# jrkerns/pylinac

Measured on AMD Instinct MI355X. Metric: EPID images/s, filter->threshold->profile->peak on 1024^2 batch, higher is better.
Workload: dtype f64

## Files before the change

pylinac_amd/csrc/hist_otsu.hip:

```cpp
#include "pl_common.h"
#include "median3_rows.h"

constexpr int kOtsuAhead = 2;

namespace {

constexpr int kHistThreads = 1024;

template <int PARTS, bool RUNS>
__global__ void __launch_bounds__(kHistThreads)
hist16_kernel(const unsigned short* __restrict__ in, int64_t n, int64_t count, unsigned flip,
              uint32_t* __restrict__ hist, const int32_t* __restrict__ only ,
              unsigned virtual_blocks) {
  constexpr int kBins = 65536 / PARTS;
  constexpr int kShift = PARTS == 4 ? 14 : 15;
  extern __shared__ unsigned bins[];
  if (only) {
    int any = 0;
    for (int64_t i = threadIdx.x; i < n; i += kHistThreads) any |= only[i];
    if (!__syncthreads_or(any)) return;
  }
  for (unsigned vb = blockIdx.x; vb < virtual_blocks; vb += gridDim.x) {
  const unsigned within = vb % (8 * PARTS);
  const int64_t frame = (int64_t)(vb / (8 * PARTS)) * 8 + (within & 7);
  const unsigned part = within >> 3;
  if (frame >= n) continue;
  if (only && !only[frame]) continue;
  __syncthreads();
  for (int i = threadIdx.x; i < kBins; i += kHistThreads) bins[i] = 0;
  __syncthreads();

  const unsigned short* src = in + frame * count;
  unsigned prev = 0xffffffffu, run = 0;
  auto tally = [&](unsigned key) {
    key ^= flip;
    if constexpr (RUNS) {
      const unsigned b = ((key >> kShift) == part) ? (key & (kBins - 1)) : 0xffffffffu;
      if (b == prev) {
        ++run;
      } else {
        if (prev != 0xffffffffu) atomicAdd(&bins[prev], run);
        prev = b;
        run = 1;
      }
    } else {
      if ((key >> kShift) == part) atomicAdd(&bins[key & (kBins - 1)], 1u);
    }
  };
  if ((reinterpret_cast<uintptr_t>(src) & 15) == 0) {
    const int64_t nvec = count / 8;
    const uint4* vsrc = reinterpret_cast<const uint4*>(src);
    auto tally4 = [&](uint4 q) {
      const unsigned first = q.x & 0xffffu;
      const unsigned splat = first | (first << 16);
      const bool lane_flat = q.x == splat && q.y == splat && q.z == splat && q.w == splat;
      const unsigned wave_first = __builtin_amdgcn_readfirstlane(splat);
      const unsigned long long active = __ballot(1);
      if (__ballot(!(lane_flat && splat == wave_first)) == 0) {
        if constexpr (!RUNS) {
          const unsigned key = (wave_first & 0xffffu) ^ flip;
          if ((key >> kShift) == part && (threadIdx.x & 63) == __builtin_ctzll(active))
            atomicAdd(&bins[key & (kBins - 1)], 8u * (unsigned)__popcll(active));
          return;
        }
      }
      const unsigned wds[4] = {q.x, q.y, q.z, q.w};
#pragma unroll
      for (int k = 0; k < 4; ++k) {
        tally(wds[k] & 0xffffu);
        tally(wds[k] >> 16);
      }
    };
    int64_t v = threadIdx.x;
    constexpr int U = 4;
    for (; v + (int64_t)(U - 1) * kHistThreads < nvec; v += (int64_t)U * kHistThreads) {
      uint4 q[U];
#pragma unroll
      for (int k = 0; k < U; ++k) q[k] = vsrc[v + (int64_t)k * kHistThreads];
#pragma unroll
      for (int k = 0; k < U; ++k) tally4(q[k]);
    }
    for (; v < nvec; v += kHistThreads) tally4(vsrc[v]);
    for (int64_t i = nvec * 8 + threadIdx.x; i < count; i += kHistThreads) tally(src[i]);
  } else {
    for (int64_t i = threadIdx.x; i < count; i += kHistThreads) tally(src[i]);
  }
  if constexpr (RUNS) {
    if (prev != 0xffffffffu) atomicAdd(&bins[prev], run);
  }
  __syncthreads();
  uint32_t* dst = hist + frame * 65536 + (size_t)part * kBins;
  for (int i = threadIdx.x; i < kBins; i += kHistThreads) dst[i] = bins[i];
  }
}

template <int PARTS, bool RUNS>
int launch_hist16(const unsigned short* in, int64_t n, int64_t count, unsigned flip, uint32_t* hist, hipStream_t st,
                  const int32_t* only = nullptr) {
  const size_t lds = (size_t)(65536 / PARTS) * sizeof(unsigned);
  static std::atomic<bool> attr{false};
  if (!attr) {
    if (hipFuncSetAttribute((const void*)hist16_kernel<PARTS, RUNS>, hipFuncAttributeMaxDynamicSharedMemorySize,
                            (int)lds) != hipSuccess) {
      (void)hipGetLastError();
      return -1;
    }
    attr = true;
  }
  const int64_t blocks = pl_cdiv(n, 8) * 8 * PARTS;
  if (blocks > 0x7fffffffLL) return -1;
  const unsigned grid = only ? (unsigned)(blocks < 256 ? blocks : 256) : (unsigned)blocks;
  hipLaunchKernelGGL((hist16_kernel<PARTS, RUNS>), dim3(grid), dim3(kHistThreads), lds, st, in, n, count,
                     flip, hist, only, (unsigned)blocks);
  return 0;
}

struct Pair { unsigned long long c; long long s; };

__device__ __forceinline__ Pair block_exclusive_scan(Pair v, Pair* total, Pair* wave_tot ) {
  const int lane = threadIdx.x & 63, wv = threadIdx.x >> 6;
  Pair inc = v;
#pragma unroll
  for (int o = 1; o < 64; o <<= 1) {
    unsigned long long c = __shfl_up(inc.c, o, 64);
    long long s = __shfl_up(inc.s, o, 64);
    if (lane >= o) { inc.c += c; inc.s += s; }
  }
  if (lane == 63) wave_tot[wv] = inc;
  __syncthreads();
  Pair base = {0, 0};
  Pair tot = {0, 0};
  for (int k = 0; k < kHistThreads / 64; ++k) {
    if (k < wv) { base.c += wave_tot[k].c; base.s += wave_tot[k].s; }
    tot.c += wave_tot[k].c; tot.s += wave_tot[k].s;
  }
  __syncthreads();
  *total = tot;
  Pair ex = {base.c + inc.c - v.c, base.s + inc.s - v.s};
  return ex;
}

__global__ void __launch_bounds__(kHistThreads)
otsu_kernel(const uint32_t* __restrict__ hist, int bias, int32_t* __restrict__ thr,
            int32_t* __restrict__ vmin, int32_t* __restrict__ vmax, const int32_t* __restrict__ only) {
  __shared__ Pair wave_tot[kHistThreads / 64];
  __shared__ int s_lo[kHistThreads / 64], s_hi[kHistThreads / 64];
  __shared__ double s_var[kHistThreads / 64];
  __shared__ int s_idx[kHistThreads / 64];
  const int64_t frame = blockIdx.x;
  if (only && !only[frame]) return;
  const uint32_t* hh = hist + frame * 65536;
  const int b0 = threadIdx.x * 64;
  const uint4* p = reinterpret_cast<const uint4*>(hh + b0);
  Pair mine = {0, 0};
  int lo = 1 << 30, hi = -1;
  for (int k4 = 0; k4 < 16; ++k4) {
    const uint4 q = p[k4];
    const uint32_t c[4] = {q.x, q.y, q.z, q.w};
#pragma unroll
    for (int j = 0; j < 4; ++j) {
      const int b = b0 + 4 * k4 + j;
      mine.c += c[j];
      mine.s += (long long)c[j] * (long long)(b - bias);
      if (c[j]) { if (lo == (1 << 30)) lo = b; hi = b; }
    }
  }
  lo = pl_wave_reduce(lo, [](int a, int b) { return a < b ? a : b; });
  hi = pl_wave_reduce(hi, [](int a, int b) { return a > b ? a : b; });
  const int lane = threadIdx.x & 63, wv = threadIdx.x >> 6;
  if (lane == 0) { s_lo[wv] = lo; s_hi[wv] = hi; }
  Pair total;
  Pair ex = block_exclusive_scan(mine, &total, wave_tot);
  for (int k = 0; k < kHistThreads / 64; ++k) { lo = s_lo[k] < lo ? s_lo[k] : lo; hi = s_hi[k] > hi ? s_hi[k] : hi; }

  double best = -1.0;
  int best_k = 1 << 30;
  double dw1 = (double)ex.c, ds1 = (double)ex.s;
  const double dW = (double)total.c, dS = (double)total.s;
  for (int k4 = 0; k4 < 16; ++k4) {
    const uint4 q = p[k4];
    const uint32_t c[4] = {q.x, q.y, q.z, q.w};
#pragma unroll
    for (int j = 0; j < 4; ++j) {
      const int b = b0 + 4 * k4 + j;
      if (c[j] != 0u) {
        dw1 += (double)c[j];
        ds1 = fma((double)c[j], (double)(b - bias), ds1);
        if (b >= lo && b < hi) {
          const double dw2 = dW - dw1;
          const double m1 = ds1 / dw1;
          const double m2 = (dS - ds1) / dw2;
          const double d = m1 - m2;
          const double var = (dw1 * dw2) * (d * d);
          if (var > best) { best = var; best_k = b; }
        }
      }
    }
  }
#pragma unroll
  for (int o = 32; o > 0; o >>= 1) {
    double ov = __shfl_xor(best, o, 64);
    int ok = __shfl_xor(best_k, o, 64);
    if (ov > best || (ov == best && ok < best_k)) { best = ov; best_k = ok; }
  }
  if (lane == 0) { s_var[wv] = best; s_idx[wv] = best_k; }
  __syncthreads();
  if (threadIdx.x == 0) {
    for (int k = 1; k < kHistThreads / 64; ++k)
      if (s_var[k] > best || (s_var[k] == best && s_idx[k] < best_k)) { best = s_var[k]; best_k = s_idx[k]; }
    thr[frame] = (lo == hi) ? (lo - bias) : (best_k - bias);
    if (vmin) vmin[frame] = lo - bias;
    if (vmax) vmax[frame] = hi - bias;
  }
}

constexpr int kWinBins = 38912;
struct OtsuScratch {
  Pair wave_tot[kHistThreads / 64];
  double s_var[kHistThreads / 64];
  int s_lo[kHistThreads / 64], s_hi[kHistThreads / 64], s_idx[kHistThreads / 64];
  int any;
};
constexpr int kOtsuScratchAt = ((kWinBins + 1) * 4 + 15) & ~15;
constexpr size_t kOtsuLds = kOtsuScratchAt + sizeof(OtsuScratch);

__device__ __forceinline__ int cell_max_see(int cm, const int (&m)[8]) {
  cm = max(max(cm, m[0]), m[1]);
  cm = max(max(cm, m[2]), m[3]);
  cm = max(max(cm, m[4]), m[5]);
  return max(max(cm, m[6]), m[7]);
}
__device__ __forceinline__ void cell_max_store(unsigned short* __restrict__ row_cells, int cm, int lane, bool on) {
  const unsigned g = pl_group8_max(on ? (unsigned)cm : 0u);
  if (on && (lane & 7) == 0) row_cells[lane >> 3] = (unsigned short)g;
}

template <typename T, bool MED3, bool CELLS>
__global__ void __launch_bounds__(kHistThreads)
otsu16_window_kernel(const unsigned short* __restrict__ in, int64_t count, int h, int w, unsigned flip, int bias,
                     const int32_t* __restrict__ lo_hint, const int32_t* __restrict__ hi_hint, int32_t* __restrict__ thr,
                     int32_t* __restrict__ vmin, int32_t* __restrict__ vmax, int32_t* __restrict__ flag, int parts,
                     uint32_t* __restrict__ merge ,
                     unsigned short* __restrict__ cellmax) {
  extern __shared__ __attribute__((aligned(16))) unsigned bins[];
  OtsuScratch& scr = *reinterpret_cast<OtsuScratch*>(reinterpret_cast<unsigned char*>(bins) + kOtsuScratchAt);
  Pair* const wave_tot = scr.wave_tot;
  int* const s_lo = scr.s_lo;
  int* const s_hi = scr.s_hi;
  double* const s_var = scr.s_var;
  int* const s_idx = scr.s_idx;
  const int64_t frame = blockIdx.x / (unsigned)parts;
  const int part = (int)(blockIdx.x % (unsigned)parts);
  const unsigned short* src = in + frame * count;
  const int lane = threadIdx.x & 63, wv = threadIdx.x >> 6;
  int klo, khi;
  if (lo_hint) {
    klo = lo_hint[frame] + bias;
    khi = hi_hint[frame] + bias;
  } else {
    int mn = 1 << 30, mx = -1;
    auto see = [&](unsigned key) {
      const int k = (int)(key ^ flip);
      mn = k < mn ? k : mn;
      mx = k > mx ? k : mx;
    };
    if ((reinterpret_cast<uintptr_t>(src) & 15) == 0 && count >= 8) {
      const int64_t nvec = count / 8;
      const uint4* vsrc = reinterpret_cast<const uint4*>(src);
      for (int64_t blk = threadIdx.x >> 7; blk * 2048 < nvec; blk += kHistThreads >> 7) {
        const int64_t idx = blk * 2048 + (threadIdx.x & 127);
        if (idx < nvec) {
          const uint4 q = vsrc[idx];
          const unsigned wds[4] = {q.x, q.y, q.z, q.w};
#pragma unroll
          for (int k = 0; k < 4; ++k) { see(wds[k] & 0xffffu); see(wds[k] >> 16); }
        }
      }
    } else {
      for (int64_t i = threadIdx.x; i < count; i += 16LL * kHistThreads) see(src[i]);
    }
    mn = pl_wave_reduce(mn, [](int a, int b) { return a < b ? a : b; });
    mx = pl_wave_reduce(mx, [](int a, int b) { return a > b ? a : b; });
    if (lane == 0) { s_lo[wv] = mn; s_hi[wv] = mx; }
    __syncthreads();
    for (int k = 0; k < kHistThreads / 64; ++k) { mn = s_lo[k] < mn ? s_lo[k] : mn; mx = s_hi[k] > mx ? s_hi[k] : mx; }
    __syncthreads();
    if (mx < mn) { mn = 0; mx = 0; }
    const int slack = kWinBins - (mx - mn + 1);
    klo = mn - (slack > 0 ? slack / 2 : 0);
    if (klo < 0) klo = 0;
    khi = klo + kWinBins - 1;
    if (khi > 65535) { khi = 65535; klo = khi - kWinBins + 1; }
    if (slack < 0) khi = klo + kWinBins;
  }
  const int range = khi - klo + 1;
  if (range > kWinBins || range <= 0 || klo < 0 || khi > 65535 || (MED3 && pl_lds_base(bins) != 0u)) {
    if (threadIdx.x == 0) flag[frame] = 1;
    return;
  }
  for (int i = threadIdx.x; i <= range; i += kHistThreads) bins[i] = 0;
  if (threadIdx.x == 0) scr.any = 0;
  __syncthreads();

  int outside = 0;
  auto tally = [&](unsigned key) {
    const unsigned b = (key ^ flip) - (unsigned)klo;
    if (b < (unsigned)range) atomicAdd(&bins[b], 1u);
    else outside = 1;
  };
  if (MED3) {
    constexpr int kRows = 32;
    constexpr int kSBias = ((T)-1 < (T)0) ? 32768 : 0;
    const unsigned kbase4 = 4u * (unsigned)(kSBias - klo);
    const int col_waves = (w / 8 + PL_WAVE - 1) / PL_WAVE, row_groups = (h + kRows - 1) / kRows;
    const int rg_lo = (int)((int64_t)row_groups * part / parts), rg_hi = (int)((int64_t)row_groups * (part + 1) / parts);
    for (int item = rg_lo * col_waves + __builtin_amdgcn_readfirstlane(wv); item < col_waves * rg_hi; item += kHistThreads / 64) {
      const int c0 = ((item % col_waves) * PL_WAVE + lane) * 8;
      const bool on = c0 < w;
      const unsigned long long act = __ballot(on);
      if (act == 0ull) continue;
      const int first_on = __builtin_ctzll(act);
      const unsigned cap4 = on ? 4u * (unsigned)range : 0u;
      const unsigned inc = on ? 1u : 0u;
      int cm = 0;
      pl_median3_rows<T, kRows, kOtsuAhead>(reinterpret_cast<const T*>(src), h, w, c0, lane, (item / col_waves) * kRows,
                             [&](int, const int (&m)[8]) {
        if constexpr (CELLS) cm = cell_max_see(cm, m);
        unsigned spread = 0;
#pragma unroll
        for (int k = 1; k < 8; ++k) spread |= (unsigned)(m[k] ^ m[0]);
        const int wave_first = __builtin_amdgcn_readlane(m[0], first_on);
        if (__ballot(on && (spread | (unsigned)(m[0] ^ wave_first)) != 0u) == 0ull) {
          const unsigned b = (unsigned)(wave_first + kSBias - klo);
          if (b < (unsigned)range) {
            if (lane == first_on) atomicAdd(&bins[b], 8u * (unsigned)__popcll(act));
          } else {
            outside = 1;
          }
          return;
        }
#pragma unroll
        for (int k = 0; k < 8; ++k) {
          const unsigned b4 = ((unsigned)m[k] << 2) + kbase4;
          const unsigned a4 = b4 < cap4 ? b4 : cap4;
          pl_lds_add_abs(a4, inc);
        }
      });
      if constexpr (CELLS) {
        const int cell_cols = (w + 63) / 64;
        cell_max_store(cellmax + ((size_t)frame * row_groups + item / col_waves) * cell_cols + (item % col_waves) * (PL_WAVE / 8), cm,
                       lane, on);
      }
    }
  } else if ((reinterpret_cast<uintptr_t>(src) & 15) == 0) {
    const int64_t nvec = count / 8;
    const uint4* vsrc = reinterpret_cast<const uint4*>(src);
    auto tally4 = [&](uint4 q) {
      const unsigned first = q.x & 0xffffu;
      const unsigned splat = first | (first << 16);
      const bool lane_flat = q.x == splat && q.y == splat && q.z == splat && q.w == splat;
      const unsigned wave_first = __builtin_amdgcn_readfirstlane(splat);
      const unsigned long long active = __ballot(1);
      if (__ballot(!(lane_flat && splat == wave_first)) == 0) {
        const unsigned b = ((wave_first & 0xffffu) ^ flip) - (unsigned)klo;
        if (b < (unsigned)range) {
          if ((threadIdx.x & 63) == __builtin_ctzll(active)) atomicAdd(&bins[b], 8u * (unsigned)__popcll(active));
        } else {
          outside = 1;
        }
        return;
      }
      const unsigned wds[4] = {q.x, q.y, q.z, q.w};
#pragma unroll
      for (int k = 0; k < 4; ++k) {
        tally(wds[k] & 0xffffu);
        tally(wds[k] >> 16);
      }
    };
    const int64_t v_lo = nvec * part / parts, v_hi = nvec * (part + 1) / parts;
    int64_t v = v_lo + threadIdx.x;
    constexpr int U = 4;
    for (; v + (int64_t)(U - 1) * kHistThreads < v_hi; v += (int64_t)U * kHistThreads) {
      uint4 q[U];
#pragma unroll
      for (int k = 0; k < U; ++k) q[k] = vsrc[v + (int64_t)k * kHistThreads];
#pragma unroll
      for (int k = 0; k < U; ++k) tally4(q[k]);
    }
    for (; v < v_hi; v += kHistThreads) tally4(vsrc[v]);
    if (part == parts - 1)
      for (int64_t i = nvec * 8 + threadIdx.x; i < count; i += kHistThreads) tally(src[i]);
  } else {
    const int64_t i_lo = count * part / parts, i_hi = count * (part + 1) / parts;
    for (int64_t i = i_lo + threadIdx.x; i < i_hi; i += kHistThreads) tally(src[i]);
  }
  if (outside) scr.any = 1;
  __syncthreads();
  const bool spilled = scr.any != 0 || (MED3 && bins[range] != 0u);
  if (parts == 1) {
    if (spilled) {
      if (threadIdx.x == 0) flag[frame] = 1;
      return;
    }
    if (threadIdx.x == 0) flag[frame] = 0;
  } else {
    uint32_t* table = merge + frame * 65536;
    unsigned seen = 0;
    if (spilled && threadIdx.x == 0) seen |= atomicExch(&flag[frame], 1) == 0x7fffffff ? 1u : 0u;
    if (!spilled)
      for (int i = threadIdx.x; i < range; i += kHistThreads) {
        const unsigned c = bins[i];
        if (c) seen |= atomicAdd(&table[i], c) == 0xffffffffu ? 1u : 0u;
      }
    if (seen) scr.any = 2;
    __syncthreads();
    if (threadIdx.x == 0) scr.any = atomicAdd(&table[65534], scr.any == 2 ? 0u : 1u) == (unsigned)(parts - 1) ? 1 : 0;
    __syncthreads();
    if (scr.any == 0) return;
    if (__hip_atomic_load(&flag[frame], __ATOMIC_RELAXED, __HIP_MEMORY_SCOPE_AGENT) != 0) return;
    for (int i = threadIdx.x; i < range; i += kHistThreads)
      bins[i] = __hip_atomic_load(&table[i], __ATOMIC_RELAXED, __HIP_MEMORY_SCOPE_AGENT);
    __syncthreads();
  }

  const int per = ((range + kHistThreads - 1) / kHistThreads) | 1;
  const int b0 = threadIdx.x * per;
  const int b1 = b0 + per < range ? b0 + per : range;
  Pair mine = {0, 0};
  int lo = 1 << 30, hi = -1;
  for (int b = b0; b < b1; ++b) {
    const unsigned c = bins[b];
    mine.c += c;
    mine.s += (long long)c * (long long)(b + klo - bias);
    if (c) { if (lo == (1 << 30)) lo = b; hi = b; }
  }
  lo = pl_wave_reduce(lo, [](int a, int b) { return a < b ? a : b; });
  hi = pl_wave_reduce(hi, [](int a, int b) { return a > b ? a : b; });
  if (lane == 0) { s_lo[wv] = lo; s_hi[wv] = hi; }
  Pair total;
  Pair ex = block_exclusive_scan(mine, &total, wave_tot);
  for (int k = 0; k < kHistThreads / 64; ++k) { lo = s_lo[k] < lo ? s_lo[k] : lo; hi = s_hi[k] > hi ? s_hi[k] : hi; }

  double best = -1.0;
  int best_k = 1 << 30;
  double dw1 = (double)ex.c, ds1 = (double)ex.s;
  const double dW = (double)total.c, dS = (double)total.s;
  for (int b = b0; b < b1; ++b) {
    const unsigned c = bins[b];
    if (c != 0u) {
      dw1 += (double)c;
      ds1 = fma((double)c, (double)(b + klo - bias), ds1);
      if (b >= lo && b < hi) {
        const double dw2 = dW - dw1;
        const double m1 = ds1 / dw1;
        const double m2 = (dS - ds1) / dw2;
        const double d = m1 - m2;
        const double var = (dw1 * dw2) * (d * d);
        if (var > best) { best = var; best_k = b; }
      }
    }
  }
#pragma unroll
  for (int o = 32; o > 0; o >>= 1) {
    double ov = __shfl_xor(best, o, 64);
    int ok = __shfl_xor(best_k, o, 64);
    if (ov > best || (ov == best && ok < best_k)) { best = ov; best_k = ok; }
  }
  if (lane == 0) { s_var[wv] = best; s_idx[wv] = best_k; }
  __syncthreads();
  if (threadIdx.x == 0) {
    for (int k = 1; k < kHistThreads / 64; ++k)
      if (s_var[k] > best || (s_var[k] == best && s_idx[k] < best_k)) { best = s_var[k]; best_k = s_idx[k]; }
    thr[frame] = (lo == hi) ? (lo + klo - bias) : (best_k + klo - bias);
    if (vmin) vmin[frame] = lo + klo - bias;
    if (vmax) vmax[frame] = hi + klo - bias;
  }
}

constexpr int kFullEvents = 2048;
constexpr int kFullBulk = 64;
struct FullScratch {
  Pair wave_tot[kHistThreads / 64];
  double s_var[kHistThreads / 64];
  int s_lo[kHistThreads / 64], s_hi[kHistThreads / 64], s_idx[kHistThreads / 64];
  int n_events, n_bulk;
  unsigned bulk_key[kFullBulk], bulk_cnt[kFullBulk];
  unsigned short event_key[kFullEvents];
};
constexpr int kFullBinsBytes = 65536 * 2;
constexpr size_t kFullLds = kFullBinsBytes + sizeof(FullScratch);

template <typename T, bool MED3, bool GUARD, bool CELLS>
__device__ __forceinline__ void full_tally_pass(const unsigned short* __restrict__ src, int64_t count, int h, int w, unsigned flip,
                                                unsigned* __restrict__ bins, FullScratch& scr,
                                                unsigned short* __restrict__ frame_cells) {
  const int lane = threadIdx.x & 63, wv = threadIdx.x >> 6;
  auto tally_n = [&](unsigned key, unsigned n) {
    const unsigned sh = (key >> 15) << 4, at = key & 0x7fffu;
    if (!GUARD) {
      pl_lds_add_abs((key << 2) & 0x1fffcu, n * (1u + ((key >> 15) & 1u) * 0xffffu));
      return;
    }
    const unsigned old = atomicAdd(&bins[at], n << sh);
    const unsigned f = (old >> sh) & 0xffffu;
    if (f < 0x8000u && f + n >= 0x8000u) {
      atomicSub(&bins[at], 0x8000u << sh);
      const int slot = atomicAdd(&scr.n_events, 1);
      if (slot < kFullEvents) scr.event_key[slot] = (unsigned short)key;
    }
  };
  auto tally = [&](unsigned key) { tally_n(key, 1u); };
  auto tally_bulk = [&](unsigned key, unsigned n, int first_on) {
    if (GUARD) {
      if (lane == first_on) tally_n(key, n);
      return;
    }
    const int have = scr.n_bulk < kFullBulk ? scr.n_bulk : kFullBulk;
    const unsigned long long hit = __ballot(lane < have && scr.bulk_key[lane] == key);
    if (lane != first_on) return;
    if (hit) { atomicAdd(&scr.bulk_cnt[__builtin_ctzll(hit)], n); return; }
    const int slot = atomicAdd(&scr.n_bulk, 1);
    if (slot < kFullBulk) { atomicAdd(&scr.bulk_cnt[slot], n); scr.bulk_key[slot] = key; }
    else tally_n(key, n);
  };
  if (MED3) {
    constexpr int kRows = 32;
    constexpr int kSBias = ((T)-1 < (T)0) ? 32768 : 0;
    const int col_waves = (w / 8 + PL_WAVE - 1) / PL_WAVE, row_groups = (h + kRows - 1) / kRows;
    for (int item = __builtin_amdgcn_readfirstlane(wv); item < col_waves * row_groups; item += kHistThreads / 64) {
      const int c0 = ((item % col_waves) * PL_WAVE + lane) * 8;
      const bool on = c0 < w;
      const unsigned long long act = __ballot(on);
      if (act == 0ull) continue;
      const int first_on = __builtin_ctzll(act);
      int cm = 0;
      pl_median3_rows<T, kRows, kOtsuAhead>(reinterpret_cast<const T*>(src), h, w, c0, lane, (item / col_waves) * kRows,
                             [&](int, const int (&m)[8]) {
        if constexpr (CELLS) cm = cell_max_see(cm, m);
        unsigned spread = 0;
#pragma unroll
        for (int k = 1; k < 8; ++k) spread |= (unsigned)(m[k] ^ m[0]);
        const int wave_first = __builtin_amdgcn_readlane(m[0], first_on);
        if (__ballot(on && (spread | (unsigned)(m[0] ^ wave_first)) != 0u) == 0ull) {
          tally_bulk((unsigned)(wave_first + kSBias), 8u * (unsigned)__popcll(act), first_on);
          return;
        }
        if (!on) return;
#pragma unroll
        for (int k = 0; k < 8; ++k) tally((unsigned)(m[k] + kSBias));
      });
      if constexpr (CELLS)
        cell_max_store(frame_cells + (size_t)(item / col_waves) * ((w + 63) / 64) + (item % col_waves) * (PL_WAVE / 8), cm, lane, on);
    }
  } else {
    for (int64_t i = threadIdx.x; i < count; i += kHistThreads) tally((unsigned)src[i] ^ flip);
  }
}

template <typename T, bool MED3, bool CELLS>
__global__ void __launch_bounds__(kHistThreads)
otsu16_full_kernel(const unsigned short* __restrict__ in, int64_t count, int h, int w, unsigned flip, int bias,
                   int32_t* __restrict__ thr, int32_t* __restrict__ vmin, int32_t* __restrict__ vmax,
                   int32_t* __restrict__ flag, unsigned short* __restrict__ cellmax) {
  extern __shared__ __attribute__((aligned(16))) unsigned bins[];
  FullScratch& scr = *reinterpret_cast<FullScratch*>(reinterpret_cast<unsigned char*>(bins) + kFullBinsBytes);
  const int64_t frame = blockIdx.x;
  if (flag[frame] == 0) return;
  const unsigned short* src = in + frame * count;
  unsigned short* frame_cells = CELLS ? cellmax + (size_t)frame * ((h + 31) / 32) * ((w + 63) / 64) : nullptr;
  const int lane = threadIdx.x & 63, wv = threadIdx.x >> 6;
  auto clear = [&]() {
    for (int i = threadIdx.x; i < 32768; i += kHistThreads) bins[i] = 0;
    if (threadIdx.x < kFullBulk) { scr.bulk_key[threadIdx.x] = 0xffffffffu; scr.bulk_cnt[threadIdx.x] = 0; }
    if (threadIdx.x == 0) { scr.n_events = 0; scr.n_bulk = 0; }
    __syncthreads();
  };

  const int b0 = threadIdx.x * 64;
  int n_events = 0, n_bulk = 0, my_notes = 0;
  auto count_of = [&](int b) {
    unsigned c = (bins[b & 0x7fff] >> ((b >> 15) << 4)) & 0xffffu;
    if (my_notes) {
      for (int e = 0; e < n_events; ++e) c += (int)scr.event_key[e] == b ? 32768u : 0u;
      for (int e = 0; e < n_bulk; ++e) c += (int)scr.bulk_key[e] == b ? scr.bulk_cnt[e] : 0u;
    }
    return c;
  };
  Pair mine, total, ex, wrapped;
  int lo, hi;
  auto totals = [&]() {
    n_events = scr.n_events < kFullEvents ? scr.n_events : kFullEvents;
    n_bulk = scr.n_bulk < kFullBulk ? scr.n_bulk : kFullBulk;
    my_notes = 0;
    for (int e = 0; e < n_events; ++e) my_notes += ((int)scr.event_key[e] >> 6) == (int)threadIdx.x ? 1 : 0;
    for (int e = 0; e < n_bulk; ++e) my_notes += (scr.bulk_key[e] >> 6) == threadIdx.x ? 1 : 0;
    mine = {0, 0};
    wrapped = {0, 0};
    lo = 1 << 30, hi = -1;
    for (int j = 0; j < 64; ++j) {
      const int b = b0 + ((j + lane) & 63);
      const unsigned c = count_of(b);
      Pair& acc = j + lane < 64 ? mine : wrapped;
      acc.c += c;
      acc.s += (long long)c * (long long)(b - bias);
      if (c) { lo = b < lo ? b : lo; hi = b > hi ? b : hi; }
    }
    mine.c += wrapped.c;
    mine.s += wrapped.s;
    lo = pl_wave_reduce(lo, [](int a, int b) { return a < b ? a : b; });
    hi = pl_wave_reduce(hi, [](int a, int b) { return a > b ? a : b; });
    if (lane == 0) { scr.s_lo[wv] = lo; scr.s_hi[wv] = hi; }
    ex = block_exclusive_scan(mine, &total, scr.wave_tot);
    for (int k = 0; k < kHistThreads / 64; ++k) { lo = scr.s_lo[k] < lo ? scr.s_lo[k] : lo; hi = scr.s_hi[k] > hi ? scr.s_hi[k] : hi; }
  };

  bool exact = false;
  if (pl_lds_base(bins) == 0u) {
    clear();
    full_tally_pass<T, MED3, false, CELLS>(src, count, h, w, flip, bins, scr, frame_cells);
    __syncthreads();
    totals();
    exact = total.c == (unsigned long long)count;
    __syncthreads();
  }
  if (!exact) {
    clear();
    full_tally_pass<T, MED3, true, CELLS>(src, count, h, w, flip, bins, scr, frame_cells);
    __syncthreads();
    totals();
  }
  double best = -1.0;
  int best_k = 1 << 30;
  double dw1 = (double)(ex.c + wrapped.c);
  double ds1 = (double)(ex.s + wrapped.s);
  const double dW = (double)total.c, dS = (double)total.s;
  for (int j = 0; j < 64; ++j) {
    if (j + lane == 64) { dw1 = (double)ex.c; ds1 = (double)ex.s; }
    const int b = b0 + ((j + lane) & 63);
    const unsigned c = count_of(b);
    if (c != 0u) {
      dw1 += (double)c;
      ds1 = fma((double)c, (double)(b - bias), ds1);
      if (b >= lo && b < hi) {
        const double dw2 = dW - dw1;
        const double m1 = ds1 / dw1;
        const double m2 = (dS - ds1) / dw2;
        const double d = m1 - m2;
        const double var = (dw1 * dw2) * (d * d);
        if (var > best || (var == best && b < best_k)) { best = var; best_k = b; }
      }
    }
  }
#pragma unroll
  for (int o = 32; o > 0; o >>= 1) {
    double ov = __shfl_xor(best, o, 64);
    int ok = __shfl_xor(best_k, o, 64);
    if (ov > best || (ov == best && ok < best_k)) { best = ov; best_k = ok; }
  }
  if (lane == 0) { scr.s_var[wv] = best; scr.s_idx[wv] = best_k; }
  __syncthreads();
  if (threadIdx.x == 0) {
    for (int k = 1; k < kHistThreads / 64; ++k)
      if (scr.s_var[k] > best || (scr.s_var[k] == best && scr.s_idx[k] < best_k)) { best = scr.s_var[k]; best_k = scr.s_idx[k]; }
    thr[frame] = (lo == hi) ? (lo - bias) : (best_k - bias);
    if (vmin) vmin[frame] = lo - bias;
    if (vmax) vmax[frame] = hi - bias;
  }
}

__global__ void __launch_bounds__(kHistThreads)
order_stats_kernel(const uint32_t* __restrict__ hist, int bias, const int64_t* __restrict__ ranks,
                   int nranks, int32_t* __restrict__ out) {
  __shared__ Pair wave_tot[kHistThreads / 64];
  const int64_t frame = blockIdx.x;
  const uint32_t* hh = hist + frame * 65536;
  const int b0 = threadIdx.x * 64;
  Pair mine = {0, 0};
  for (int k = 0; k < 64; ++k) mine.c += hh[b0 + k];
  Pair total;
  Pair ex = block_exclusive_scan(mine, &total, wave_tot);
  for (int q = 0; q < nranks; ++q) {
    long long r = ranks[q];
    if (r < 0) r = 0;
    if ((unsigned long long)r >= total.c) r = (long long)total.c - 1;
    if ((unsigned long long)r >= ex.c && (unsigned long long)r < ex.c + mine.c) {
      unsigned long long acc = ex.c;
      for (int k = 0; k < 64; ++k) {
        acc += hh[b0 + k];
        if ((unsigned long long)r < acc) { out[frame * nranks + q] = b0 + k - bias; break; }
      }
    }
  }
}


constexpr int kTwBinsWide = 19456, kTwBinsWl = 9728;
struct TwScratch { int s_lo[kHistThreads / 64], s_hi[kHistThreads / 64]; };
constexpr int tw_scratch_at(int bins) { return (2 * bins + 1 + PL_WAVE + 3) / 4 * 16; }
constexpr size_t tw_lds(int bins) { return tw_scratch_at(bins) + sizeof(TwScratch); }

template <int kTwBins, int WAVES_PER_EU>
__global__ void __launch_bounds__(kHistThreads, WAVES_PER_EU)
hist16_two_window_kernel(const unsigned short* __restrict__ in, int64_t count, unsigned flip, uint32_t* __restrict__ hist,
                         unsigned short* __restrict__ tile_max , int eh, int ew, int ews,
                         int32_t* __restrict__ edge_min, int32_t* __restrict__ edge_max ,
                         const int64_t* __restrict__ ranks, int nranks, int32_t* __restrict__ stats ) {
  extern __shared__ __attribute__((aligned(16))) unsigned bins[];
  TwScratch& scr = *reinterpret_cast<TwScratch*>(reinterpret_cast<unsigned char*>(bins) + tw_scratch_at(kTwBins));
  const int64_t frame = blockIdx.x;
  const unsigned short* src = in + frame * count;
  uint32_t* row = hist + frame * 65536;
  const int lane = threadIdx.x & 63, wv = threadIdx.x >> 6;
  const bool vec = (reinterpret_cast<uintptr_t>(src) & 15) == 0 && count >= 8;
  const int64_t nvec = vec ? count / 8 : 0;
  const uint4* vsrc = reinterpret_cast<const uint4*>(src);

  for (int i = threadIdx.x; i < 2 * kTwBins; i += kHistThreads) bins[i] = 0;
  if (edge_min) {
    int mn = 0x7fffffff, mx = -0x7fffffff - 1;
    auto value = [&](unsigned short raw) { return flip ? (int)(short)raw : (int)raw; };
    auto see = [&](int v) { mn = v < mn ? v : mn; mx = v > mx ? v : mx; };
    const int band = ews < eh ? ews : eh, cb = ews < ew ? ews : ew;
    constexpr int E = 4;
    for (int e0 = threadIdx.x; e0 < band * ew; e0 += E * kHistThreads) {
      unsigned short a[E], b[E];
#pragma unroll
      for (int k = 0; k < E; ++k) {
        const int e = e0 + k * kHistThreads < band * ew ? e0 + k * kHistThreads : e0;
        a[k] = src[e];
        b[k] = src[(int64_t)(eh - band) * ew + e];
      }
#pragma unroll
      for (int k = 0; k < E; ++k) { see(value(a[k])); see(value(b[k])); }
    }
    for (int e0 = threadIdx.x; e0 < eh * cb; e0 += E * kHistThreads) {
      unsigned short a[E], b[E];
#pragma unroll
      for (int k = 0; k < E; ++k) {
        const int e = e0 + k * kHistThreads < eh * cb ? e0 + k * kHistThreads : e0;
        const int r = e / cb, c = e - r * cb;
        a[k] = src[(int64_t)r * ew + c];
        b[k] = src[(int64_t)r * ew + (ew - cb) + c];
      }
#pragma unroll
      for (int k = 0; k < E; ++k) { see(value(a[k])); see(value(b[k])); }
    }
    mn = pl_wave_reduce(mn, [](int a, int b) { return a < b ? a : b; });
    mx = pl_wave_reduce(mx, [](int a, int b) { return a > b ? a : b; });
    if (lane == 0) { scr.s_lo[wv] = mn; scr.s_hi[wv] = mx; }
    __syncthreads();
    if (threadIdx.x == 0) {
      for (int k = 0; k < kHistThreads / 64; ++k) { mn = scr.s_lo[k] < mn ? scr.s_lo[k] : mn; mx = scr.s_hi[k] > mx ? scr.s_hi[k] : mx; }
      edge_min[frame] = mn;
      edge_max[frame] = mx;
    }
    __syncthreads();
  }
  const int64_t ntiles = (count + 511) / 512;
  unsigned short* const tmax = tile_max ? tile_max + frame * ntiles : nullptr;
  if (tmax)
    for (int64_t i = threadIdx.x; i < ntiles; i += kHistThreads) tmax[i] = (unsigned short)0xffffu;
  int mn = 1 << 30, mx = -1;
  auto see = [&](unsigned key) {
    const int k = (int)(key ^ flip);
    mn = k < mn ? k : mn;
    mx = k > mx ? k : mx;
  };
  if (vec) {
    for (int64_t blk = threadIdx.x >> 7; blk * 2048 < nvec; blk += kHistThreads >> 7) {
      const int64_t idx = blk * 2048 + (threadIdx.x & 127);
      if (idx < nvec) {
        const uint4 q = vsrc[idx];
        const unsigned wds[4] = {q.x, q.y, q.z, q.w};
#pragma unroll
        for (int k = 0; k < 4; ++k) { see(wds[k] & 0xffffu); see(wds[k] >> 16); }
      }
    }
  } else {
    for (int64_t i = threadIdx.x; i < count; i += 16LL * kHistThreads) see(src[i]);
  }
  mn = pl_wave_reduce(mn, [](int a, int b) { return a < b ? a : b; });
  mx = pl_wave_reduce(mx, [](int a, int b) { return a > b ? a : b; });
  if (lane == 0) { scr.s_lo[wv] = mn; scr.s_hi[wv] = mx; }
  __syncthreads();
  for (int k = 0; k < kHistThreads / 64; ++k) { mn = scr.s_lo[k] < mn ? scr.s_lo[k] : mn; mx = scr.s_hi[k] > mx ? scr.s_hi[k] : mx; }
  if (mx < mn) { mn = 0; mx = 0; }
  int w0, w1;
  if (mx - mn + 1 <= 2 * kTwBins) {
    w0 = mn - (2 * kTwBins - (mx - mn + 1)) / 2;
    w0 = w0 < 0 ? 0 : (w0 > 65536 - 2 * kTwBins ? 65536 - 2 * kTwBins : w0);
    w1 = w0 + kTwBins;
  } else {
    w0 = mn - 256 < 0 ? 0 : mn - 256;
    w1 = mx + 256 > 65535 ? 65536 - kTwBins : mx + 257 - kTwBins;
    if (w1 < w0 + kTwBins) w1 = w0 + kTwBins;
  }
  const unsigned uw0 = (unsigned)w0, uw1 = (unsigned)w1;
  for (int i = threadIdx.x; i < 65536 / 4; i += kHistThreads) {
    const unsigned b = 4u * (unsigned)i;
    const bool inside = (b - uw0 < (unsigned)kTwBins && b + 3u - uw0 < (unsigned)kTwBins) ||
                        (b - uw1 < (unsigned)kTwBins && b + 3u - uw1 < (unsigned)kTwBins);
    if (!inside) reinterpret_cast<uint4*>(row)[i] = uint4{0u, 0u, 0u, 0u};
  }
  __syncthreads();

  unsigned hot = 0;
  unsigned guess = 0xffffffffu;
  auto add_key = [&](unsigned key, unsigned n) {
    const unsigned b0 = key - uw0, b1 = key - uw1;
    if (b0 < (unsigned)kTwBins) atomicAdd(&bins[b0], n);
    else if (b1 < (unsigned)kTwBins) atomicAdd(&bins[kTwBins + b1], n);
    else atomicAdd(row + key, n);
  };
  auto flush = [&]() {
    const unsigned tot = pl_wave_reduce(hot, [](unsigned a, unsigned b) { return a + b; });
    if (tot != 0u && lane == 0) add_key(guess, tot);
    hot = 0;
    return tot;
  };
  const unsigned base = pl_lds_base(bins);
  const unsigned k0 = base - 4u * uw0, k1 = base + 4u * (unsigned)kTwBins - 4u * uw1;
  const unsigned spare_addr = base + 4u * (unsigned)(2 * kTwBins), dummy_addr = spare_addr + 4u + 4u * (unsigned)lane;
  auto tally = [&](unsigned raw, unsigned long long& outside) {
    const unsigned key = raw ^ flip;
    const bool in0 = key - uw0 < (unsigned)kTwBins, in1 = key - uw1 < (unsigned)kTwBins, is_hot = key == guess;
    unsigned addr = in0 ? (key << 2) + k0 : (in1 ? (key << 2) + k1 : spare_addr);
    addr = is_hot ? dummy_addr : addr;
    hot += is_hot ? 1u : 0u;
    pl_lds_add_abs(addr, 1u);
    outside |= __ballot(!(in0 || in1 || is_hot));
  };
  auto tally4 = [&](uint4 q) {
    const unsigned first = q.x & 0xffffu;
    const unsigned splat = first | (first << 16);
    const bool lane_flat = q.x == splat && q.y == splat && q.z == splat && q.w == splat;
    const unsigned wave_first = __builtin_amdgcn_readfirstlane(splat);
    const unsigned long long active = __ballot(1);
    if (__ballot(!(lane_flat && splat == wave_first)) == 0) {
      if ((threadIdx.x & 63) == __builtin_ctzll(active)) add_key((wave_first & 0xffffu) ^ flip, 8u * (unsigned)__popcll(active));
// ... 364 lines not shown
```

pylinac_amd/csrc/median3_rows.h:

```cpp
#pragma once

template <typename T, int ROWS, int AHEAD = 4, bool BYOFFSET = false, typename F>
__device__ __forceinline__ void pl_median3_rows(const T* __restrict__ f, int h, int w, int c0, int lane, int r0_lane, F&& consume,
                                                bool load = true) {
  static_assert(sizeof(T) == 2, "16-bit dtypes");
  const int r0 = __builtin_amdgcn_readfirstlane(r0_lane);
  const bool active = c0 < w;
  const unsigned offc = (unsigned)(active ? c0 : 0) * 2u;
  const bool first = c0 == 0, last = c0 + 8 >= w;
  const bool edge_l = lane == 0 && !first, edge_r = lane == PL_WAVE - 1 && !last && active;
  const bool edge = edge_l || edge_r;
  const unsigned offe = edge_l ? offc - 2u : offc + 16u;
  struct Raw { uint4 q; int e; };
  [[maybe_unused]] __amdgpu_buffer_rsrc_t rs;
  [[maybe_unused]] unsigned voffq = 0, voffe = 0;
  if constexpr (BYOFFSET) {
    rs = pl_make_rsrc_bounded(f, (unsigned)h * (unsigned)w * 2u);
    voffq = load ? offc : kPlBufferNowhere;
    voffe = load && edge ? offe : kPlBufferNowhere;
  }
  auto fetch = [&](int r) {
    const int rm = 2 * h - 1 - r;
    int rr = r < rm ? r : rm;
    rr = rr > 0 ? rr : 0;
    const char* row = reinterpret_cast<const char*>(f) + (size_t)rr * (size_t)w * 2u;
    Raw x{uint4{0u, 0u, 0u, 0u}, 0};
    if constexpr (BYOFFSET) {
      const unsigned soff = (unsigned)rr * (unsigned)w * 2u;
      x.q = pl_buffer_load_u128(rs, voffq, soff);
      x.e = (int)pl_buffer_load_u16(rs, voffe, soff);
    } else if (load) {
      x.q = *reinterpret_cast<const uint4*>(row + offc);
      x.e = edge ? (int)*reinterpret_cast<const T*>(row + offe) : 0;
    }
    return x;
  };
  int lo[3][8], mi[3][8], hi[3][8];
  auto digest = [&](const Raw& x, int slot) {
    const unsigned wd[4] = {x.q.x, x.q.y, x.q.z, x.q.w};
    int xe = x.e;
    if constexpr (BYOFFSET) xe = pl_extend16_here<T>(x.e);
    int v[10];
#pragma unroll
    for (int k = 0; k < 4; ++k) {
      v[1 + 2 * k] = (int)(T)(wd[k] & 0xffffu);
      v[2 + 2 * k] = (int)(T)(wd[k] >> 16);
    }
    const int left = __builtin_amdgcn_update_dpp(xe, v[8], 0x138, 0xf, 0xf, false);
    const int right = __builtin_amdgcn_update_dpp(xe, v[1], 0x130, 0xf, 0xf, false);
    v[0] = first ? v[1] : left;
    v[9] = last ? v[8] : right;
#pragma unroll
    for (int j = 0; j < 8; ++j) {
      const int a = v[j], b = v[j + 1], c = v[j + 2];
      lo[slot][j] = min(min(a, b), c);
      hi[slot][j] = max(max(a, b), c);
      mi[slot][j] = pl_smed3(a, b, c);
    }
  };
  auto emit = [&](int k) {
    const int r = r0 + k - 2;
    if (r >= h) return;
    int m[8];
#pragma unroll
    for (int j = 0; j < 8; ++j)
      m[j] = pl_smed3(max(max(lo[0][j], lo[1][j]), lo[2][j]), pl_smed3(mi[0][j], mi[1][j], mi[2][j]),
                      min(min(hi[0][j], hi[1][j]), hi[2][j]));
    consume(r, m);
  };
  Raw ring[AHEAD];
#pragma unroll
  for (int k = 0; k < AHEAD; ++k) ring[k] = fetch(r0 - 1 + k);
  constexpr int kChunk = (AHEAD % 3 == 0) ? AHEAD : 3 * AHEAD;
  auto step = [&](int k, int ring_slot, int tri_slot) {
    const Raw cur = ring[ring_slot];
    ring[ring_slot] = fetch(r0 - 1 + k + AHEAD);
    digest(cur, tri_slot);
  };
  step(0, 0 % AHEAD, 0);
  step(1, 1 % AHEAD, 1);
  constexpr int kMain = (ROWS / kChunk) * kChunk;
#pragma unroll 1
  for (int kb = 2; kb < 2 + kMain; kb += kChunk) {
#pragma unroll
    for (int j = 0; j < kChunk; ++j) {
      step(kb + j, (2 + j) % AHEAD, (2 + j) % 3);
      emit(kb + j);
    }
  }
#pragma unroll
  for (int k = 2 + kMain; k < ROWS + 2; ++k) {
    step(k, k % AHEAD, k % 3);
    emit(k);
  }
}

__device__ __forceinline__ unsigned pl_pack16(int a, int b) { return ((unsigned)a & 0xffffu) | ((unsigned)b << 16); }

static inline bool pl_median3_rows_covers(const void* in, int h, int w) {
  return h > 1 && w >= 8 && (w & 7) == 0 && (reinterpret_cast<uintptr_t>(in) & 15) == 0 && (((size_t)h * w) & 7) == 0;
}
static inline bool pl_median3_rows_bounded_covers(int h, int w) { return (int64_t)h * (int64_t)w * 2 < (int64_t)kPlBufferNowhere; }
```

Measured before the change: 389,200.

## Stream median3 rows over multi-group spans per wave in windowed Otsu histogram

The windowed Otsu kernel now gives each wave a contiguous span of several 32-row groups instead of one group per item. The median3 row pipeline gets a SPAN mode that walks a variable row count with buffer-offset loads and prefetch depth 3, so the halo rows reloaded per group and the pipeline warm-up cost are amortised. The min/max sampling pass batches eight vector loads before consuming them, and bin zeroing is overlapped with those loads. Cell-max stores are now issued at group boundaries inside the span, and the out-of-range flag goes to shared scratch; this adds register pressure and a new size guard for buffer addressing.

```diff
diff --git a/pylinac_amd/csrc/hist_otsu.hip b/pylinac_amd/csrc/hist_otsu.hip
--- a/pylinac_amd/csrc/hist_otsu.hip
+++ b/pylinac_amd/csrc/hist_otsu.hip
@@ -1,7 +1,8 @@
 #include "pl_common.h"
 #include "median3_rows.h"
 
-constexpr int kOtsuAhead = 2;
+constexpr int kOtsuAhead = 3;
+constexpr int kOtsuFullAhead = 2;
 
 namespace {
 
@@ -254,9 +255,14 @@
   const unsigned short* src = in + frame * count;
   const int lane = threadIdx.x & 63, wv = threadIdx.x >> 6;
   int klo, khi;
+  auto zero_bins = [&]() {
+    for (int i = threadIdx.x; i <= kWinBins; i += kHistThreads) bins[i] = 0;
+    if (threadIdx.x == 0) scr.any = 0;
+  };
   if (lo_hint) {
     klo = lo_hint[frame] + bias;
     khi = hi_hint[frame] + bias;
+    zero_bins();
   } else {
     int mn = 1 << 30, mx = -1;
     auto see = [&](unsigned key) {
@@ -267,16 +273,27 @@
     if ((reinterpret_cast<uintptr_t>(src) & 15) == 0 && count >= 8) {
       const int64_t nvec = count / 8;
       const uint4* vsrc = reinterpret_cast<const uint4*>(src);
-      for (int64_t blk = threadIdx.x >> 7; blk * 2048 < nvec; blk += kHistThreads >> 7) {
-        const int64_t idx = blk * 2048 + (threadIdx.x & 127);
-        if (idx < nvec) {
-          const uint4 q = vsrc[idx];
-          const unsigned wds[4] = {q.x, q.y, q.z, q.w};
+      constexpr int kSample = 8;
+      constexpr int64_t kBlkStep = kHistThreads >> 7;
+      bool zeroed = false;
+      for (int64_t blk = threadIdx.x >> 7; blk * 2048 < nvec; blk += kSample * kBlkStep) {
+        uint4 q[kSample];
+#pragma unroll
+        for (int s = 0; s < kSample; ++s) {
+          const int64_t idx = (blk + s * kBlkStep) * 2048 + (threadIdx.x & 127);
+          q[s] = vsrc[idx < nvec ? idx : 0];
+        }
+        if (!zeroed) { zero_bins(); zeroed = true; }
+#pragma unroll
+        for (int s = 0; s < kSample; ++s) {
+          const unsigned wds[4] = {q[s].x, q[s].y, q[s].z, q[s].w};
 #pragma unroll
           for (int k = 0; k < 4; ++k) { see(wds[k] & 0xffffu); see(wds[k] >> 16); }
         }
       }
+      if (!zeroed) zero_bins();
     } else {
+      zero_bins();
       for (int64_t i = threadIdx.x; i < count; i += 16LL * kHistThreads) see(src[i]);
     }
     mn = pl_wave_reduce(mn, [](int a, int b) { return a < b ? a : b; });
@@ -294,12 +311,11 @@
     if (slack < 0) khi = klo + kWinBins;
   }
   const int range = khi - klo + 1;
-  if (range > kWinBins || range <= 0 || klo < 0 || khi > 65535 || (MED3 && pl_lds_base(bins) != 0u)) {
+  if (range > kWinBins || range <= 0 || klo < 0 || khi > 65535 ||
+      (MED3 && (pl_lds_base(bins) != 0u || (int64_t)h * (int64_t)w * 2 >= (int64_t)kPlBufferNowhere))) {
     if (threadIdx.x == 0) flag[frame] = 1;
     return;
   }
-  for (int i = threadIdx.x; i <= range; i += kHistThreads) bins[i] = 0;
-  if (threadIdx.x == 0) scr.any = 0;
   __syncthreads();
 
   int outside = 0;
@@ -310,22 +326,29 @@
   };
   if (MED3) {
     constexpr int kRows = 32;
+    constexpr int kWaves = kHistThreads / 64;
     constexpr int kSBias = ((T)-1 < (T)0) ? 32768 : 0;
     const unsigned kbase4 = 4u * (unsigned)(kSBias - klo);
     const int col_waves = (w / 8 + PL_WAVE - 1) / PL_WAVE, row_groups = (h + kRows - 1) / kRows;
     const int rg_lo = (int)((int64_t)row_groups * part / parts), rg_hi = (int)((int64_t)row_groups * (part + 1) / parts);
-    for (int item = rg_lo * col_waves + __builtin_amdgcn_readfirstlane(wv); item < col_waves * rg_hi; item += kHistThreads / 64) {
-      const int c0 = ((item % col_waves) * PL_WAVE + lane) * 8;
+    const int groups = rg_hi - rg_lo;
+    const int per_block = groups * col_waves <= kWaves ? groups : (col_waves < kWaves ? kWaves / col_waves : 1);
+    for (int span = __builtin_amdgcn_readfirstlane(wv); span < per_block * col_waves; span += kWaves) {
+      const int cb = span % col_waves, run = span / col_waves;
+      const int g0 = rg_lo + (int)((int64_t)groups * run / per_block), g1 = rg_lo + (int)((int64_t)groups * (run + 1) / per_block);
+      const int c0 = (cb * PL_WAVE + lane) * 8;
       const bool on = c0 < w;
       const unsigned long long act = __ballot(on);
       if (act == 0ull) continue;
       const int first_on = __builtin_ctzll(act);
-      const unsigned cap4 = on ? 4u * (unsigned)range : 0u;
+      const unsigned cap4 = 4u * (unsigned)range;
       const unsigned inc = on ? 1u : 0u;
       int cm = 0;
-      pl_median3_rows<T, kRows, kOtsuAhead>(reinterpret_cast<const T*>(src), h, w, c0, lane, (item / col_waves) * kRows,
-                             [&](int, const int (&m)[8]) {
-        if constexpr (CELLS) cm = cell_max_see(cm, m);
+      [[maybe_unused]] const int cell_cols = (w + 63) / 64;
+      [[maybe_unused]] unsigned short* const cells =
+          CELLS ? cellmax + (size_t)frame * row_groups * cell_cols + cb * (PL_WAVE / 8) : nullptr;
+      [[maybe_unused]] const int r_last = (g1 * kRows < h ? g1 * kRows : h) - 1;
+      auto tally_row = [&](const int (&m)[8]) {
         unsigned spread = 0;
 #pragma unroll
         for (int k = 1; k < 8; ++k) spread |= (unsigned)(m[k] ^ m[0]);
@@ -335,7 +358,7 @@
           if (b < (unsigned)range) {
             if (lane == first_on) atomicAdd(&bins[b], 8u * (unsigned)__popcll(act));
           } else {
-            outside = 1;
+            if (lane == first_on) scr.any = 1;
           }
           return;
         }
@@ -345,12 +368,18 @@
           const unsigned a4 = b4 < cap4 ? b4 : cap4;
           pl_lds_add_abs(a4, inc);
         }
-      });
-      if constexpr (CELLS) {
-        const int cell_cols = (w + 63) / 64;
-        cell_max_store(cellmax + ((size_t)frame * row_groups + item / col_waves) * cell_cols + (item % col_waves) * (PL_WAVE / 8), cm,
-                       lane, on);
-      }
+      };
+      pl_median3_rows<T, kRows, kOtsuAhead, true, true>(reinterpret_cast<const T*>(src), h, w, c0, lane, g0 * kRows,
+                             [&](int r, const int (&m)[8]) {
+        if constexpr (CELLS) cm = cell_max_see(cm, m);
+        tally_row(m);
+        if constexpr (CELLS) {
+          if ((r & (kRows - 1)) == kRows - 1 || r == r_last) {
+            cell_max_store(cells + (size_t)(r / kRows) * cell_cols, cm, lane, on);
+            cm = 0;
+          }
+        }
+      }, true, (g1 - g0) * kRows);
     }
   } else if ((reinterpret_cast<uintptr_t>(src) & 15) == 0) {
     const int64_t nvec = count / 8;
@@ -534,7 +563,7 @@
       if (act == 0ull) continue;
       const int first_on = __builtin_ctzll(act);
       int cm = 0;
-      pl_median3_rows<T, kRows, kOtsuAhead>(reinterpret_cast<const T*>(src), h, w, c0, lane, (item / col_waves) * kRows,
+      pl_median3_rows<T, kRows, kOtsuFullAhead>(reinterpret_cast<const T*>(src), h, w, c0, lane, (item / col_waves) * kRows,
                              [&](int, const int (&m)[8]) {
         if constexpr (CELLS) cm = cell_max_see(cm, m);
         unsigned spread = 0;
diff --git a/pylinac_amd/csrc/median3_rows.h b/pylinac_amd/csrc/median3_rows.h
--- a/pylinac_amd/csrc/median3_rows.h
+++ b/pylinac_amd/csrc/median3_rows.h
@@ -1,10 +1,15 @@
 #pragma once
 
-template <typename T, int ROWS, int AHEAD = 4, bool BYOFFSET = false, typename F>
+template <typename T, int ROWS, int AHEAD = 4, bool BYOFFSET = false, bool SPAN = false, typename F>
 __device__ __forceinline__ void pl_median3_rows(const T* __restrict__ f, int h, int w, int c0, int lane, int r0_lane, F&& consume,
-                                                bool load = true) {
+                                                bool load = true, int rows_lane = ROWS) {
   static_assert(sizeof(T) == 2, "16-bit dtypes");
   const int r0 = __builtin_amdgcn_readfirstlane(r0_lane);
+  [[maybe_unused]] int r_stop = h;
+  if constexpr (SPAN) {
+    const int r_end = r0 + __builtin_amdgcn_readfirstlane(rows_lane);
+    r_stop = r_end < h ? r_end : h;
+  }
   const bool active = c0 < w;
   const unsigned offc = (unsigned)(active ? c0 : 0) * 2u;
   const bool first = c0 == 0, last = c0 + 8 >= w;
@@ -60,7 +65,11 @@
   };
   auto emit = [&](int k) {
     const int r = r0 + k - 2;
-    if (r >= h) return;
+    if constexpr (SPAN) {
+      if (r >= r_stop) return;
+    } else {
+      if (r >= h) return;
+    }
     int m[8];
 #pragma unroll
     for (int j = 0; j < 8; ++j)
@@ -73,12 +82,29 @@
   for (int k = 0; k < AHEAD; ++k) ring[k] = fetch(r0 - 1 + k);
   constexpr int kChunk = (AHEAD % 3 == 0) ? AHEAD : 3 * AHEAD;
   auto step = [&](int k, int ring_slot, int tri_slot) {
+    if constexpr (SPAN) {
+      digest(ring[ring_slot], tri_slot);
+      ring[ring_slot] = fetch(r0 - 1 + k + AHEAD);
+      return;
+    }
     const Raw cur = ring[ring_slot];
     ring[ring_slot] = fetch(r0 - 1 + k + AHEAD);
     digest(cur, tri_slot);
   };
   step(0, 0 % AHEAD, 0);
   step(1, 1 % AHEAD, 1);
+  if constexpr (SPAN) {
+    const int k_end = 2 + (r_stop - r0);
+#pragma unroll 1
+    for (int kb = 2; kb < k_end; kb += kChunk) {
+#pragma unroll
+      for (int j = 0; j < kChunk; ++j) {
+        step(kb + j, (2 + j) % AHEAD, (2 + j) % 3);
+        emit(kb + j);
+      }
+    }
+    return;
+  }
   constexpr int kMain = (ROWS / kChunk) * kChunk;
 #pragma unroll 1
   for (int kb = 2; kb < 2 + kMain; kb += kChunk) {
```

Result: no change. 387,600 (-0.4%).
